# Chemical118/TREW

Measured on AMD Instinct MI355X. Metric: Gbases/s scanned (short 5 32, 150 bp reads), higher is better.
Workload: dtype u32

## Files before the change

### include/trew_hip.h

```cpp
#ifndef TREW_HIP_H
#define TREW_HIP_H

#include <stddef.h>
#include <stdint.h>

#ifdef __cplusplus
extern "C" {
#endif

#define TREW_HIP_ABI_VERSION 4

enum {
    TREW_MODE_SHORT = 0,
    TREW_MODE_PAIR = 1,
    TREW_MODE_LONG = 2,
    TREW_MODE_SEGMENT = 3
};

enum {
    TREW_TABLE_FORWARD_HIGH = 0,
    TREW_TABLE_FORWARD_LOW = 1,
    TREW_TABLE_BACKWARD_HIGH = 2,
    TREW_TABLE_BACKWARD_LOW = 3,
    TREW_TABLE_BOTH_HIGH = 4,
    TREW_TABLE_BOTH_LOW = 5,
    TREW_NUM_TABLES = 6
};

enum {
    TREW_FLAG_NO_FILTER = 1,
    TREW_FLAG_DEBUG_NO_EMIT = 2,
    TREW_FLAG_DEBUG_NO_KLOOP = 4,
    TREW_FLAG_DEBUG_POISON_LDS = 32,
    TREW_FLAG_DEBUG_WIDE_NO_WAIT = 128,
    TREW_FLAG_NO_TIMING = 64,
    TREW_FLAG_COMPAT_G1 = 512,
    TREW_FLAG_DEBUG_NO_JOINT = 2048,
    TREW_FLAG_DEBUG_NO_UNI_DRAIN = 4096,
    TREW_FLAG_DEBUG_NO_GROUP = 1024,
    TREW_FLAG_DEBUG_ANNOT_GENERAL = 8192,
    TREW_FLAG_TRACK_PRESSURE = 256
};

typedef struct {
    int32_t min_mer;
    int32_t max_mer;
    double low_baseline;
    double high_baseline;
    int32_t slice_length;
    int32_t mode;
    int32_t device;
    int32_t n_slots;
    uint64_t max_batch_words;
    uint64_t max_batch_reads;
    uint32_t table_log2_slots;
    uint32_t flags;
    uint64_t max_batch_ascii_bytes;
} trew_hip_params;

typedef struct {
    const uint32_t *words;
    uint64_t n_words;
    const uint32_t *offsets;
    const uint32_t *lengths;
    uint32_t uniform_length;
    uint32_t uniform_stride;
    uint64_t n_reads;
    int32_t on_device;
    int32_t max_length;
} trew_hip_batch;

typedef struct {
    const char *bases;
    uint64_t n_bytes;
    const uint32_t *byte_offsets;
    const uint32_t *lengths;
    const uint32_t *word_offsets;
    uint32_t uniform_length;
    uint32_t reserved;
    uint64_t n_reads;
} trew_hip_ascii_batch;

typedef struct {
    int32_t k;
    int32_t table;
    uint64_t word_lo;
    uint64_t word_hi;
    uint64_t count;
} trew_hip_row;

typedef struct trew_hip_ctx trew_hip_ctx;

int trew_hip_init(const trew_hip_params *params, trew_hip_ctx **out);
void trew_hip_destroy(trew_hip_ctx *ctx);
const char *trew_hip_last_error(const trew_hip_ctx *ctx);

int trew_hip_submit(trew_hip_ctx *ctx, const trew_hip_batch *batch, int slot);
int trew_hip_submit_ascii(trew_hip_ctx *ctx, const trew_hip_ascii_batch *batch, int slot);
int trew_hip_pack_ascii(trew_hip_ctx *ctx, const trew_hip_ascii_batch *batch, uint32_t *words, uint64_t words_cap, uint64_t *n_words);
int trew_hip_wait(trew_hip_ctx *ctx, int slot);

int trew_hip_collect(trew_hip_ctx *ctx, int table, trew_hip_row *rows, uint64_t cap, uint64_t *n_rows);
int trew_hip_reset_tables(trew_hip_ctx *ctx);
int trew_hip_add_rows(trew_hip_ctx *ctx, const trew_hip_row *rows, uint64_t n_rows);

int trew_hip_collect_device(trew_hip_ctx *ctx, trew_hip_row *d_rows, uint64_t cap, uint64_t *n_rows);
int trew_hip_add_rows_device(trew_hip_ctx *ctx, const trew_hip_row *d_rows, uint64_t n_rows);
int trew_hip_merge(trew_hip_ctx *dst, trew_hip_ctx *src);
int trew_hip_add_gathered_device(trew_hip_ctx *ctx, const trew_hip_row *d_buf, uint32_t n_slices, uint32_t own_slice,
                                 uint64_t slice_rows, void *producer_stream, uint64_t *max_rows);
int trew_hip_collect_slice_device(trew_hip_ctx *ctx, trew_hip_row *d_slice, uint64_t slice_rows, void *consumer_stream, uint64_t *n_rows);

int trew_hip_table_pressure(trew_hip_ctx *ctx, uint64_t *used_slots, uint64_t *total_slots, uint64_t *spilled_rows,
                            uint64_t *spill_capacity);

#define TREW_DEBUG_COUNTERS 8
int trew_hip_debug_counters(trew_hip_ctx *ctx, uint64_t *out, int n);

int trew_hip_debug_worklist(trew_hip_ctx *ctx, int slot, uint32_t *units, uint64_t cap, uint64_t *n);

int trew_hip_segment_results(trew_hip_ctx *ctx, int slot, int32_t *k_high, int32_t *k_low,
                             uint64_t *seq_high, uint64_t *seq_low, uint64_t *seq_high_hi, uint64_t *seq_low_hi,
// ... 88 lines not shown
```

### trew_amd/__init__.py

```python
from . import capi
from .capi import (
    FLAG_NO_FILTER,
    FLAG_DEBUG_ANNOT_GENERAL,
    FLAG_DEBUG_POISON_LDS,
    FLAG_NO_TIMING,
    FLAG_TRACK_PRESSURE,
    FLAG_COMPAT_G1,
    FLAG_DEBUG_NO_GROUP,
    FLAG_DEBUG_NO_JOINT,
    FLAG_DEBUG_NO_UNI_DRAIN,
    FLAG_DEBUG_WIDE_NO_WAIT,
    MODE_LONG,
    MODE_PAIR,
    MODE_SEGMENT,
    MODE_SHORT,
    TABLE_NAMES,
    TrewHip,
    TrewHipError,
    annotate,
    intervals,
    k_mer_check,
    pack_reads,
    tracts,
    variants,
)
```

### trew_amd/capi.py

```python
from __future__ import annotations

import ctypes as C
import os

import numpy as np

_HERE = os.path.dirname(os.path.abspath(__file__))
LIB_PATH = os.environ.get("TREW_HIP_LIB") or os.path.join(_HERE, "lib", "libtrew_hip.so")

MODE_SHORT, MODE_PAIR, MODE_LONG, MODE_SEGMENT = 0, 1, 2, 3
FLAG_NO_FILTER = 1
FLAG_DEBUG_POISON_LDS = 32
FLAG_NO_TIMING = 64
FLAG_COMPAT_G1 = 512
FLAG_TRACK_PRESSURE = 256
FLAG_DEBUG_NO_JOINT = 2048
FLAG_DEBUG_NO_UNI_DRAIN = 4096
FLAG_DEBUG_NO_GROUP = 1024
FLAG_DEBUG_ANNOT_GENERAL = 8192
FLAG_DEBUG_WIDE_NO_WAIT = 128
TABLE_NAMES = ("forward_high", "forward_low", "backward_high", "backward_low", "both_high", "both_low")

EXPORTED_SYMBOLS = (
    "trew_hip_init", "trew_hip_destroy", "trew_hip_last_error", "trew_hip_submit", "trew_hip_wait",
    "trew_hip_collect", "trew_hip_reset_tables", "trew_hip_add_rows", "trew_hip_segment_results",
    "trew_hip_filter_masks", "trew_hip_last_timing", "trew_pack_words", "trew_pack_reads",
    "trew_synth_short_ascii", "trew_synth_short_device", "trew_synth_pair_ascii", "trew_synth_pair_device",
    "trew_hip_malloc", "trew_hip_free", "trew_hip_memcpy_h2d", "trew_hip_memcpy_d2h", "trew_hip_abi_version",
    "trew_pack_pairs", "trew_hip_host_alloc", "trew_hip_host_free", "trew_hip_device_count",
    "trew_synth_long_lengths", "trew_synth_long_ascii", "trew_synth_long_device",
    "trew_hip_collect_device", "trew_hip_add_rows_device", "trew_hip_merge", "trew_hip_table_pressure",
    "trew_hip_add_gathered_device", "trew_hip_collect_slice_device", "trew_hip_debug_counters", "trew_hip_debug_worklist", "trew_hip_submit_ascii", "trew_hip_pack_ascii",
    "trew_motif_parse", "trew_hip_annotate", "trew_hip_annotate_results", "trew_annotate_host",
    "trew_hip_tracts", "trew_hip_tracts_results", "trew_tracts_host",
    "trew_hip_intervals", "trew_hip_intervals_results", "trew_intervals_host",
    "trew_hip_variants", "trew_hip_variants_results", "trew_variants_host",
)
DEBUG_COUNTERS = ("strict_rerun", "windows_fallback", "wide_spin_timeout", "inserted", "inserted_wide", "group_punt", "group_routed", "group_target")


class Params(C.Structure):
    _fields_ = [
        ("min_mer", C.c_int32), ("max_mer", C.c_int32),
        ("low_baseline", C.c_double), ("high_baseline", C.c_double),
        ("slice_length", C.c_int32), ("mode", C.c_int32), ("device", C.c_int32), ("n_slots", C.c_int32),
        ("max_batch_words", C.c_uint64), ("max_batch_reads", C.c_uint64),
        ("table_log2_slots", C.c_uint32), ("flags", C.c_uint32),
        ("max_batch_ascii_bytes", C.c_uint64),
    ]


class Batch(C.Structure):
    _fields_ = [
        ("words", C.c_void_p), ("n_words", C.c_uint64),
        ("offsets", C.c_void_p), ("lengths", C.c_void_p),
        ("uniform_length", C.c_uint32), ("uniform_stride", C.c_uint32),
        ("n_reads", C.c_uint64), ("on_device", C.c_int32), ("max_length", C.c_int32),
    ]


class AsciiBatch(C.Structure):
    _fields_ = [
        ("bases", C.c_void_p), ("n_bytes", C.c_uint64),
        ("byte_offsets", C.c_void_p), ("lengths", C.c_void_p), ("word_offsets", C.c_void_p),
        ("uniform_length", C.c_uint32), ("reserved", C.c_uint32), ("n_reads", C.c_uint64),
    ]


class Row(C.Structure):
    _fields_ = [("k", C.c_int32), ("table", C.c_int32), ("word_lo", C.c_uint64), ("word_hi", C.c_uint64),
                ("count", C.c_uint64)]


class Motif(C.Structure):
    _fields_ = [("k", C.c_int32), ("reserved", C.c_int32), ("word", C.c_uint64)]


class Annot(C.Structure):
    _fields_ = [("windows_fwd", C.c_uint32), ("windows_rev", C.c_uint32), ("tract_start_fwd", C.c_uint32),
                ("tract_len_fwd", C.c_uint32), ("tract_start_rev", C.c_uint32), ("tract_len_rev", C.c_uint32)]


ANNOT_DTYPE = np.dtype([(name, "<u4") for name, _ in Annot._fields_])
assert ANNOT_DTYPE.itemsize == C.sizeof(Annot)
MAX_MOTIFS = 8


class Tract(C.Structure):
    _fields_ = [(name + sfx, C.c_uint32) for sfx in ("_fwd", "_rev")
                for name in ("covered", "head_len", "head_cov", "tail_len", "tail_cov")]


TRACT_DTYPE = np.dtype([(name, "<u4") for name, _ in Tract._fields_])
assert TRACT_DTYPE.itemsize == C.sizeof(Tract) == 40


class IntervalRule(C.Structure):
    _fields_ = [("max_gap", C.c_uint32), ("min_len", C.c_uint32)]


class Interval(C.Structure):
# ... 637 lines not shown
```

### trew_amd/csrc/kernels/decide_group.inc

```

#define TREW_REGION_LIST(X) \
    X(chunk) X(stage) X(group_setup) X(bounds) X(group) X(dg_loop) X(dg_pick) X(dg_eval) X(er_gaps) X(er_runs) X(er_canon) X(er_merge) X(er_max) \
    X(dg_decision) X(dg_end) X(routing) X(records) X(target) X(target_rows) X(target_eval) X(target_emit) X(fallback)
#define TREW_REGION_ENUM(n) kRegion_##n,
enum { TREW_REGION_LIST(TREW_REGION_ENUM) kRegionCount };
#ifdef TREW_REGION_COUNTS
__device__ unsigned long long g_region[64];
#define TREW_MARK(n)                                                                   \
    do {                                                                               \
        asm volatile("; MARK " #n);                                                    \
        if (lane_id() == 0) atomicAdd(&g_region[kRegion_##n], 1ull);                   \
    } while (0)
#else
#define TREW_MARK(n) asm volatile("; MARK " #n)
#endif
__device__ __forceinline__ void lds_sync() {
    __builtin_amdgcn_fence(__ATOMIC_RELEASE, "wavefront");
    __builtin_amdgcn_wave_barrier();
    __builtin_amdgcn_fence(__ATOMIC_ACQUIRE, "wavefront");
}
#define TREW_DPP(v, ctrl) ((u32) __builtin_amdgcn_update_dpp(0, (int) (v), (ctrl), 0xf, 0xf, false))
__device__ __forceinline__ u32 swap16(u32 v) { return (u32) __builtin_amdgcn_ds_swizzle((int) v, 0x401F); }
template <int G = 16>
__device__ __forceinline__ u32 row_or(u32 v) {
// ... 3 lines not shown
    v |= TREW_DPP(v, 0x121);
    if (G == 32) v |= swap16(v);
    return v;
}
template <int G = 16>
__device__ __forceinline__ u32 row_add(u32 v) {
    v += TREW_DPP(v, 0x128);
    v += TREW_DPP(v, 0x124);
    v += TREW_DPP(v, 0x122);
    v += TREW_DPP(v, 0x121);
    if (G == 32) v += swap16(v);
    return v;
}
template <int G = 16>
__device__ __forceinline__ u32 row_max(u32 v) {
    v = max(v, TREW_DPP(v, 0x128));
    v = max(v, TREW_DPP(v, 0x124));
    v = max(v, TREW_DPP(v, 0x122));
    v = max(v, TREW_DPP(v, 0x121));
    if (G == 32) v = max(v, swap16(v));
    return v;
}
__device__ __forceinline__ u32 lane_gather(u32 v, u32 src) { return (u32) __builtin_amdgcn_ds_bpermute((int) (src << 2), (int) v); }
__device__ __forceinline__ u64 lane_gather(u64 v, u32 src) { return ((u64) lane_gather((u32) (v >> 32), src) << 32) | lane_gather((u32) v, src); }

template <int NW>
__device__ __forceinline__ u32 pack_bound(const LaneMasks<NW> &m, const DevParams &P) {
    static_assert(NW <= 10, "COUNT must fit 10 bits");
    const u32 runs = m.runs < 127u ? m.runs : 127u;
    return m.m8 | (m.cnt << 10) | (runs << 20) | (m.ub >= P.low ? 1u << 27 : 0u) | (m.ub >= P.high ? 1u << 28 : 0u) | (m.has_n ? 1u << 29 : 0u);
}

__device__ __forceinline__ void group_fill_multiples(ExactSmem sm, const DevParams &P) {
    const u32 i = lane_id();
    if (i < 32u) {
        const int k = P.min_mer + (int) i;
        u32 m = 0;
        for (int t = k; t <= P.min_mer + 31; t += k) m |= 1u << (t - P.min_mer);
        sm_group(sm)[kGroupMult + i] = m;
    }
}

template <int NW>
__device__ __forceinline__ u32 select_bit(const u32 (&m)[NW], u32 r) {
    u32 word = m[0], sub = 0, base = 0, cum = 0;
#pragma unroll
    for (int w = 0; w + 1 < NW; w++) {
        cum += __popc(m[w]);
        const bool ge = r >= cum;
        word = ge ? m[w + 1] : word;
        sub = ge ? cum : sub;
        base = ge ? 32u * (u32) (w + 1) : base;
    }
    r -= sub;
#pragma unroll
    for (u32 sh = 16; sh >= 1; sh >>= 1) {
        const u32 c = __popc(word & ((1u << sh) - 1u));
        const bool ge = r >= c;
        r -= ge ? c : 0u;
        word = ge ? word >> sh : word;
        base += ge ? sh : 0u;
    }
    return base;
}

__device__ __forceinline__ u64 window_word_at(ExactSmem sm, u32 p, int k) {
    const u32 wi = p >> 5, sh = 2u * (p & 31u);
    const u64 a = sm_seq(sm)[wi], b = sm_seq(sm)[wi + 1];
    const u64 x = sh ? ((a << sh) | (b >> (64u - sh))) : a;
    return x >> (64 - 2 * k);
}

template <typename WT>
struct RowCount {
    u32 R;
    u32 over;
    u32 count;
    WT canon;
    u32 cnt;
    u32 maxc;
    u32 homo;
    WT mseq;
};
template <int NW, typename WT, bool WANT_SEQ, int G = 16>
__device__ __forceinline__ RowCount<WT> eval_row(ExactSmem sm, const u32 (&lo)[NW], const u32 (&hi)[NW], const u32 (&v1)[NW], u32 has_n, u32 s0, int k,
                                                 int W, u32 ev) {
    static_assert(G == 16 || G == 32, "a group is a DPP row or half a wave");
    constexpr u32 kGM = G == 32 ? 0xffffffffu : 0xffffu;
    const u32 lane = lane_id(), j = lane & (u32) (G - 1), gbase = lane & (u32) (64 - G);
    RowCount<WT> rc;
    u32 V[NW];
#pragma unroll
    for (int w = 0; w < NW; w++) {
        V[w] = low_mask(W - 32 * w);
    }
    u32 many_n = 0;
    const bool gaps = __any((ev & has_n) != 0u);
    if (gaps) {
        TREW_MARK(er_gaps);
        u32 nn[NW], left = 0;
#pragma unroll
        for (int w = 0; w < NW; w++) {
            nn[w] = (ev & has_n) ? (~v1[w] & low_mask(W + k - 1 - 32 * w)) : 0u;
            left += __popc(nn[w]);
        }
        many_n = left > 4u ? 1u : 0u;
        left = many_n ? 0u : left;
        while (__any(left != 0u)) {
            u32 p = 0, found = 0;
#pragma unroll
            for (int w = 0; w < NW; w++) {
                const u32 here = (found == 0u && nn[w] != 0u) ? 1u : 0u;
                p = here ? 32u * (u32) w + (u32) __builtin_ctz(nn[w] | (here ^ 1u)) : p;
                nn[w] = here ? (nn[w] & (nn[w] - 1u)) : nn[w];
                found |= here;
            }
            const int a = left ? ((int) p - k + 1 > 0 ? (int) p - k + 1 : 0) : 0, b = left ? (int) p + 1 : 0;
#pragma unroll
            for (int w = 0; w < NW; w++) {
                V[w] &= ~(low_mask(b - 32 * w) & ~low_mask(a - 32 * w));
            }
            left = left ? left - 1u : 0u;
        }
    }
    TREW_MARK(er_runs);
    u32 st[NW], E[NW], R = 0, count = 0;
    {
        u32 prev = 0;
#pragma unroll
        for (int w = 0; w < NW; w++) {
            E[w] = ~((lo[w] ^ shr_var_word<NW>(lo, w, (u32) k)) | (hi[w] ^ shr_var_word<NW>(hi, w, (u32) k)));
            const u32 ve = V[w] & E[w];
            st[w] = V[w] & ~((ve << 1) | (prev >> 31));
            prev = ve;
            R += __popc(st[w]);
            count += __popc(V[w]);
        }
    }
    rc.R = R;
    rc.count = count;
    rc.over = ev & ((R > (u32) G ? 1u : 0u) | many_n);
    ev &= rc.over ^ 1u;
    const bool runlane = ev != 0u && j < R;
    const u32 s = runlane ? select_bit<NW>(st, j) : 0u;
    u32 e;
    if (gaps) {
        u32 en[NW];
#pragma unroll
        for (int w = 0; w < NW; w++) {
            const u32 vn = w + 1 < NW ? V[w + 1 < NW ? w + 1 : 0] : 0u;
            en[w] = V[w] & ~(E[w] & alignbit(vn, V[w], 1u));
        }
        e = runlane ? select_bit<NW>(en, j) : 0u;
    } else {
        const u32 nxt = G == 32 ? (u32) __builtin_amdgcn_update_dpp(0, (int) s, 0x130, 0xf, 0xf, true) : (u32) __builtin_amdgcn_update_dpp(0, (int) s, 0x101, 0xf, 0xf, true);
        e = (j + 1u < R) ? nxt - 1u : (u32) (W - 1);
    }
    const u32 len = e - s + 1u;
    WT canon = ~(WT) 0;
    TREW_MARK(er_canon);
    if (runlane) canon = min_rotation<WT>(window_word_at(sm, s0 + s, k), k);
    u32 rem = ev ? (R >= (u32) G ? kGM : ((1u << (R & 31u)) - 1u)) : 0u;
    u32 tot = 0, last = 0, first = 0;
    u32 covered = 0, best = 0;
    while (__any(rem != 0u)) {
        TREW_MARK(er_merge);
        const bool open = ((rem >> j) & 1u) != 0u;
        const u32 lead = rem ? (u32) __builtin_ctz(rem) : 0u;
        const WT other = lane_gather(canon, gbase + lead);
        const bool eq = open && other == canon;
        const u32 bal = (u32) (__ballot(eq) >> gbase) & kGM;
        const u32 total = row_add<G>(eq ? len : 0u);
        const u32 lend = lane_gather(e, gbase + (bal ? 31u - (u32) __builtin_clz(bal) : 0u));
        covered += total;
        best = total > best ? total : best;
        const bool settled = rem != 0u && best > count - covered;
        const bool alone = settled && open && !eq;
        tot = eq ? total : (alone ? len : tot);
        last = eq ? lend : (alone ? e : last);
        first = eq ? (j == lead ? 1u : 0u) : (alone ? 1u : first);
        rem = settled ? 0u : (rem & ~bal);
    }
    TREW_MARK(er_max);
    const u32 key = runlane ? ((tot << 16) | (0xffffu - last)) : 0u;
    const u32 mkey = row_max<G>(key);
    const u32 win = (runlane && key == mkey) ? 1u : 0u;
    rc.maxc = mkey >> 16;
    rc.homo = row_or<G>(win & (is_homopolymer<WT>(canon, k) ? 1u : 0u));
    rc.mseq = 0;
    if (WANT_SEQ) {
        const u32 wb = (u32) (__ballot(win != 0u) >> gbase) & kGM;
        rc.mseq = lane_gather(canon, gbase + (wb ? (u32) __builtin_ctz(wb) : 0u));
    }
    rc.canon = canon;
    rc.cnt = first ? tot : 0u;
    return rc;
}

template <int NW, int G = 16, bool IN_LDS = true>
__device__ __forceinline__ void row_prepare(ExactSmem sm, const ReadRef &rd, const Segment &sg, bool rowvalid) {
    static_assert((64 / G) * 6 * NW <= 128, "the groups' 6 NW words each must fit kGroupBnd's 128 words");
    static_assert(3 * NW <= G, "a lane per (feature, word)");
    const u32 lane = lane_id(), g = lane / (u32) G, j = lane & (u32) (G - 1);
    u32 *prep = sm_group(sm) + kGroupBnd + g * (6u * NW);
    const u32 p = j / (u32) NW, w = j - p * (u32) NW;
    const bool mine = j < 3u * NW && rowvalid;
    u32 lo1[1] = {0}, hi1[1] = {0}, nm1[1] = {0};
    if (mine) {
        if (IN_LDS)
            load_planes_lds<1>(rd, sg.start + 32u * w, lo1, hi1, nm1);
        else
            load_planes<1>(rd, sg.start + 32u * w, lo1, hi1, nm1);
    }
    const u32 v1 = ~nm1[0] & low_mask((int) sg.len - 32 * (int) w);
    const u32 f1 = lo1[0] & v1, f2 = hi1[0] & v1;
    const u32 x = word_parity(p == 0u ? f1 : (p == 1u ? f2 : (f1 & f2)));
    const u32 top = mine ? x >> 31 : 0u;
    u32 carry = 0;
#pragma unroll
    for (int u = 0; u + 1 < NW; u++) {
        const u32 t = lane_gather(top, g * (u32) G + p * (u32) NW + (u32) u);
        carry ^= (u32) u < w ? t : 0u;
    }
    if (mine) {
        prep[j] = p == 0u ? lo1[0] : (p == 1u ? hi1[0] : v1);
        prep[3 * NW + j] = ((x ^ (0u - carry)) << 1) | carry;
    }
}

template <int NW>
struct RowSeg {
    u32 lo[NW], hi[NW], v1[NW], P1[NW], P2[NW], P3[NW];
    u32 has_n;
};
template <int NW, int G = 16>
__device__ __forceinline__ void row_load(ExactSmem sm, int L, RowSeg<NW> &r) {
    const u32 g = lane_id() / (u32) G;
    const u32 *prep = sm_group(sm) + kGroupBnd + g * (6u * NW);
    u32 anyn = 0;
#pragma unroll
    for (int w = 0; w < NW; w++) {
        r.lo[w] = prep[0 * NW + w];
        r.hi[w] = prep[1 * NW + w];
        r.v1[w] = prep[2 * NW + w];
        r.P1[w] = prep[3 * NW + w];
        r.P2[w] = prep[4 * NW + w];
        r.P3[w] = prep[5 * NW + w];
        anyn |= ~r.v1[w] & low_mask(L - 32 * w);
    }
    r.has_n = anyn != 0u ? 1u : 0u;
}

template <int NW, bool SMALLK>
__device__ __forceinline__ u32 shr_k_word(const u32 (&x)[NW], int w, u32 k) {
    if (SMALLK) return alignbit(w + 1 < NW ? x[w + 1 < NW ? w + 1 : 0] : 0u, x[w], k);
    return shr_var_word<NW>(x, w, k);
}
template <int NW, bool SMALLK = false>
__device__ __forceinline__ u32 bound_at_k(const RowSeg<NW> &r, int L, int k, int gmax, const DevParams &P) {
    const u32 ku = (u32) k;
    u32 V[NW];
    windows_without_n<NW>(r.v1, r.has_n != 0u , L, k, 32, V);
    Buckets8<false, false> b8;
    u32 Ew[NW];
#pragma unroll
    for (int w = 0; w < NW; w++) {
        const u32 F1 = r.P1[w] ^ shr_k_word<NW, SMALLK>(r.P1, w, ku), F2 = r.P2[w] ^ shr_k_word<NW, SMALLK>(r.P2, w, ku);
        const u32 F3 = r.P3[w] ^ shr_k_word<NW, SMALLK>(r.P3, w, ku);
        Ew[w] = ~((r.lo[w] ^ shr_k_word<NW, SMALLK>(r.lo, w, ku)) | (r.hi[w] ^ shr_k_word<NW, SMALLK>(r.hi, w, ku)));
        b8.add(F1, F2, F3, V[w]);
    }
    const u32 m8 = b8.largest(), count = b8.count, links = class_links<NW>(V, Ew);
    const u32 runs = count - links < 127u ? count - links : 127u;
    const double dm = (double) m8, dc = (double) count;
    const double tl = P.low * dc, th = P.high * dc;
    u32 pass_lo = dm > tl ? 1u : 0u, pass_hi = dm > th ? 1u : 0u;
    const bool amb = fabs(dm - tl) <= 1e-9 || fabs(dm - th) <= 1e-9;
    if (__any(amb)) {
        const double ub = count ? dm / dc : 0.0;
        pass_lo = ub >= P.low ? 1u : 0u;
        pass_hi = ub >= P.high ? 1u : 0u;
    }
    const bool inr = k <= gmax && count != 0u;
    return inr ? (m8 | (count << 10) | (runs << 20) | (pass_lo << 27) | (pass_hi << 28) | (r.has_n << 29)) : (r.has_n << 29);
}

template <typename WT>
struct GroupOut {
    u32 kk;
    WT sh, sl;
    u32 saved;
    WT kept_canon;
    u32 kept_cnt;
    bool punt;
};

template <int NW, typename WT, bool WANT_SEQ, int G = 16>
__device__ __forceinline__ GroupOut<WT> decide_group(ExactSmem sm, const DevParams &P, const RowSeg<NW> &rs, u32 bnd0, u32 bnd1, u32 range, const Segment &sg,
                                                     bool valid) {
    static_assert(sizeof(WT) == 8, "k <= 32: the k range must fit a 32-bit index mask");
    PH_T0(t_ph);
    const u32 lane = lane_id(), j = lane & (u32) (G - 1), gbase = lane & (u32) (64 - G);
    const u32 *grp = sm_group(sm);
    const u32 (&lo)[NW] = rs.lo;
    const u32 (&hi)[NW] = rs.hi;
    const int L = (int) sg.len;
    const u32 s0 = range_base(sm, range) + sg.start;
    const u32 has_n = rs.has_n;
    GroupOut<WT> o;
    o.kk = 0;
    o.sh = o.sl = 0;
    o.saved = 0;
    o.kept_canon = 0;
    o.kept_cnt = 0;
    u32 todo = 0;
    {
        const u32 a = (u32) (sg.kmin - P.min_mer) & 31u, b = (u32) (sg.kmax - P.min_mer);
        const u32 m = (b >= 31u ? 0xffffffffu : ((2u << (b & 31u)) - 1u)) & ~((1u << a) - 1u);
        todo = (valid && sg.kmax >= sg.kmin) ? m : 0u;
    }
    u32 lo_num = 0, lo_den = 0, hi_num = 0, hi_den = 0, closed_lo = 0, closed_hi = 0;
    u32 sk0 = 0, sk1 = 0, skb0 = 0, skb1 = 0, skm0 = 0, skm1 = 0;
    u32 viol = 0, punt = 0;
    const u32 m8_0 = bnd0 & 1023u, cn_0 = (bnd0 >> 10) & 1023u, m8_1 = bnd1 & 1023u, cn_1 = (bnd1 >> 10) & 1023u;
    const u32 bit0 = 1u << j, bit1 = G == 16 ? 1u << ((16u + j) & 31u) : 0u;
    auto eligible = [&]() __attribute__((always_inline)) -> u32 {
        const u32 l0 = (bnd0 >> 27) & ~(closed_lo >> j) & (__umul24(m8_0, lo_den) >= __umul24(lo_num, cn_0) ? 1u : 0u);
        const u32 h0 = (bnd0 >> 28) & ~(closed_hi >> j) & (__umul24(m8_0, hi_den) >= __umul24(hi_num, cn_0) ? 1u : 0u);
        if (G == 32) return row_or<G>(((l0 | h0) & 1u) ? bit0 : 0u);
        const u32 l1 = (bnd1 >> 27) & ~(closed_lo >> ((16u + j) & 31u)) & (__umul24(m8_1, lo_den) >= __umul24(lo_num, cn_1) ? 1u : 0u);
        const u32 h1 = (bnd1 >> 28) & ~(closed_hi >> ((16u + j) & 31u)) & (__umul24(m8_1, hi_den) >= __umul24(hi_num, cn_1) ? 1u : 0u);
        return row_or<G>((((l0 | h0) & 1u) ? bit0 : 0u) | (((l1 | h1) & 1u) ? bit1 : 0u));
    };
    TREW_MARK(dg_loop);
    todo &= eligible();
    for (;;) {
        u32 act, kidx, bk;
        for (;;) {
            TREW_MARK(dg_pick);
            act = (todo != 0u && punt == 0u) ? 1u : 0u;
            kidx = act ? (u32) __builtin_ctz(todo) : 0u;
            bk = G == 32 ? lane_gather(bnd0, gbase + kidx) : lane_gather(kidx >= 16u ? bnd1 : bnd0, gbase + (kidx & 15u));
            const u32 heavy = act & (((bk >> 20) & 127u) > (u32) G ? 1u : 0u);
            if (!__any(heavy)) break;
            const u32 m8k = bk & 1023u, cntk = (bk >> 10) & 1023u;
            const u32 el = ((bk >> 27) & ~(closed_lo >> kidx) & (__umul24(m8k, lo_den) >= __umul24(lo_num, cntk) ? 1u : 0u) & 1u) |
                           (((bk >> 28) & ~(closed_hi >> kidx) & (__umul24(m8k, hi_den) >= __umul24(hi_num, cntk) ? 1u : 0u) & 1u) << 1);
            const u32 mk = grp[kGroupMult + kidx];
            const u32 take0 = heavy & (sk0 == 0u ? 1u : 0u), take1 = heavy & (take0 ^ 1u) & (sk1 == 0u ? 1u : 0u);
            sk0 = take0 ? (kidx | (el << 8) | (1u << 12)) : sk0;
            skb0 = take0 ? (m8k | (cntk << 16)) : skb0;
            skm0 = take0 ? mk : skm0;
            sk1 = take1 ? (kidx | (el << 8) | (1u << 12)) : sk1;
            skb1 = take1 ? (m8k | (cntk << 16)) : skb1;
            skm1 = take1 ? mk : skm1;
            punt |= heavy & ((take0 | take1) ^ 1u);
            todo = heavy ? (todo & (todo - 1u)) : todo;
        }
        if (!__any(act)) break;
        TREW_MARK(dg_eval);
        todo &= todo - 1u;
        const int k = P.min_mer + (int) kidx;
        const u32 lo_open = ~(closed_lo >> kidx) & 1u, hi_open = ~(closed_hi >> kidx) & 1u;
        u32 ev = act;
        const int W = ev ? L - k + 1 : 1;
        PH_T0(t_runs);
        const RowCount<WT> rc = eval_row<NW, WT, WANT_SEQ, G>(sm, lo, hi, rs.v1, has_n, s0, k, W, ev);
        punt |= rc.over;
        ev &= rc.over ^ 1u;
        const u32 R = rc.R, maxc = rc.maxc, count = rc.count, homo = rc.homo;
        const WT mseq = rc.mseq, canon = rc.canon;
        PH_ADD(PH_RUNS, t_runs);
        TREW_MARK(dg_decision);
        const double dm = (double) maxc, dc = (double) count;
        const double tl = P.low * dc, th = P.high * dc;
        u32 base_lo = dm > tl ? 1u : 0u, base_hi = dm > th ? 1u : 0u;
        if (__any(ev != 0u && (fabs(dm - tl) <= 1e-9 || fabs(dm - th) <= 1e-9))) {
            const double f = dm / dc;
            base_lo = f >= P.low ? 1u : 0u;
            base_hi = f >= P.high ? 1u : 0u;
        }
        const u32 ge_lo = lo_den ? (__umul24(maxc, lo_den) >= __umul24(lo_num, count) ? 1u : 0u) : base_lo;
        const u32 ge_hi = hi_den ? (__umul24(maxc, hi_den) >= __umul24(hi_num, count) ? 1u : 0u) : base_hi;
        const u32 okv = ev & (homo ^ 1u) & (maxc != 0u ? 1u : 0u);
        const u32 acc_lo = okv & lo_open & ge_lo, acc_hi = okv & hi_open & ge_hi, acc = acc_lo | (acc_hi << 1);
        const u32 mk = grp[kGroupMult + kidx];
        o.kk = acc_lo ? ((o.kk & 0xffu) | ((u32) k << 8)) : o.kk;
        o.kk = acc_hi ? ((o.kk & 0xff00u) | (u32) k) : o.kk;
        lo_num = acc_lo ? maxc : lo_num;
        lo_den = acc_lo ? count : lo_den;
        hi_num = acc_hi ? maxc : hi_num;
        hi_den = acc_hi ? count : hi_den;
        closed_lo |= acc_lo ? mk : 0u;
        closed_hi |= acc_hi ? mk : 0u;
        if (WANT_SEQ) {
            o.sl = acc_lo ? mseq : o.sl;
            o.sh = acc_hi ? mseq : o.sh;
        }
        o.saved = acc ? ((u32) k | (R << 8) | (count << 16)) : o.saved;
        o.kept_canon = acc ? canon : o.kept_canon;
        o.kept_cnt = acc ? rc.cnt : o.kept_cnt;
        {
            const u32 hit0 = acc & (sk0 >> 8) & 3u, hit1 = acc & (sk1 >> 8) & 3u;
            const u32 bad0 = (__umul24(maxc, skb0 >> 16) < __umul24(skb0 & 0xffffu, count) ? 1u : 0u) | ((skm0 >> kidx) & 1u);
            const u32 bad1 = (__umul24(maxc, skb1 >> 16) < __umul24(skb1 & 0xffffu, count) ? 1u : 0u) | ((skm1 >> kidx) & 1u);
            viol |= (hit0 ? bad0 : 0u) | (hit1 ? bad1 : 0u);
            sk0 |= hit0 << 10;
            sk1 |= hit1 << 10;
        }
        if (__any(acc)) {
            todo &= eligible();
            if (!__any(todo != 0u && punt == 0u)) break;
        }
    }
    TREW_MARK(dg_end);
    viol |= ((sk0 >> 8) & 3u & ~((sk0 >> 10) & 3u)) | ((sk1 >> 8) & 3u & ~((sk1 >> 10) & 3u));
    o.punt = (punt | viol) != 0u;
    PH_ADD(PH_DECIDE, t_ph);
    return o;
}

__device__ __forceinline__ void stage_two(ExactSmem sm, const ReadRef &rdA, const ReadRef &rdB, bool haveB) {
    const u32 lane = lane_id();
    lds_sync();
    const u32 r = lane >> 5, segwords = exact_rangewords(sm.cap);
    ReadRef rr;
    rr.w = r ? rdB.w : rdA.w;
    rr.len = r ? rdB.len : rdA.len;
    rr.nw = r ? rdB.nw : rdA.nw;
    const u32 L = rr.len;
    u64 *seq = sm_seq(sm) + r * segwords;
    u32 *nmk = sm_nmask(sm) + r * segwords;
    const u32 nwords = (L + 31u) >> 5;
    if (r == 0u || haveB) {
        for (u32 l = lane & 31u; l < segwords; l += 32u) {
            u64 sq = 0;
            u32 nmv = 0xffffffffu;
            if (l < nwords) {
                u32 lo1[1], hi1[1], nm1[1];
                load_planes_lds<1>(rr, 32u * l, lo1, hi1, nm1);
                nmv = nm1[0] | ~low_mask<true>((int) L - 32 * (int) l);
                const u32 lq = lo1[0] & ~nmv, hq = hi1[0] & ~nmv;
                sq = spread32(__brev(lq)) | (spread32(__brev(hq)) << 1);
            }
            seq[l] = sq;
            nmk[l] = nmv;
        }
    }
    lds_sync();
}

template <typename WT>
__device__ __forceinline__ WT strand_canon(WT w, int k) {
    const WT rc = min_rotation<WT>(revcomp(w, k), k);
    return rc < w ? rc : w;
}

template <typename WT>
__device__ __forceinline__ WT strand_flip(WT w, int k) {
    return min_rotation<WT>(revcomp(w, k), k);
}

template <int NW, typename WT>
__device__ void run_short_group(ExactSmem sm, const DevParams &P, TableRef T, const ReadRef rdA, const ReadRef rdB, bool haveB) {
    const u32 lane = lane_id();
#if defined(TREW_AB_SKIP) && TREW_AB_SKIP >= 5
    return;
#endif
    TREW_MARK(stage);
    PH_T0(t_stage);
    stage_two(sm, rdA, rdB, haveB);
    PH_ADD(PH_STAGE, t_stage);
#if defined(TREW_AB_SKIP) && TREW_AB_SKIP >= 4
    return;
#endif
    TREW_MARK(group_setup);
    const u32 g = lane >> 4, j = lane & 15u;
    const bool second = g >= 2u;
    const u32 is_right = g & 1u;
    ReadRef rd;
    rd.w = second ? rdB.w : rdA.w;
    rd.len = second ? rdB.len : rdA.len;
    rd.nw = second ? rdB.nw : rdA.nw;
    const Segment sg = get_segment(TREW_MODE_SHORT, (int) is_right, rd.len, 0, P.min_mer, P.max_mer, P.slice_len);
    const bool rowvalid = sg.valid && (!second || haveB);
    TREW_MARK(bounds);
    PH_T0(t_bounds);
    lds_sync();
    row_prepare<NW>(sm, rd, sg, rowvalid);
    lds_sync();
    RowSeg<NW> rs;
    row_load<NW>(sm, (int) sg.len, rs);
    u32 bnd0;
    if (P.min_mer + 15 < 32)
        bnd0 = rowvalid ? bound_at_k<NW, true>(rs, (int) sg.len, P.min_mer + (int) j, P.max_mer, P) : 0u;
    else
        bnd0 = rowvalid ? bound_at_k<NW, false>(rs, (int) sg.len, P.min_mer + (int) j, P.max_mer, P) : 0u;
    const u32 bnd1 = rowvalid ? bound_at_k<NW>(rs, (int) sg.len, P.min_mer + 16 + (int) j, P.max_mer, P) : 0u;
#if defined(TREW_AB_SKIP) && TREW_AB_SKIP >= 3
    asm volatile("" ::"v"(bnd0), "v"(bnd1));
    return;
#endif
    PH_ADD(PH_BOUNDS, t_bounds);
    TREW_MARK(group);
    const GroupOut<WT> o = decide_group<NW, WT, false>(sm, P, rs, bnd0, bnd1, second ? 1u : 0u, sg, rowvalid);
#if defined(TREW_AB_SKIP) && TREW_AB_SKIP >= 2
    asm volatile("" ::"v"(o.kk), "v"(o.saved), "v"(o.kept_cnt), "v"((u32) o.kept_canon), "v"((u32) (o.kept_canon >> 32)), "v"((u32) o.punt));
    return;
#endif
    TREW_MARK(routing);
    PH_T0(t_route);
    const u32 mine = rowvalid ? (o.kk | (o.punt ? 1u << 16 : 0u)) : 0u;
    const u32 other = lane_gather(mine, lane ^ 16u);
    const u32 kkL = is_right ? other : mine, kkR = is_right ? mine : other;
    const u32 lkh = kkL & 255u, lkl = (kkL >> 8) & 255u, rkh = kkR & 255u, rkl = (kkR >> 8) & 255u;
    const u32 left_found = (lkh | lkl) != 0u ? 1u : 0u;
    const u32 tgt_h = left_found & (lkh == rkh ? 1u : 0u) & (lkh != 0u ? 1u : 0u);
    const u32 tgt_l = left_found & (lkl == rkl ? 1u : 0u) & (lkl != 0u ? 1u : 0u);
    const u32 myk = o.saved & 255u, items = (o.saved >> 8) & 255u;
    u32 need_old = ((kkL | kkR) >> 16) & 1u;
    u32 rec_mask = 0;
    {
        const u32 kh = is_right ? rkh : lkh, kl = is_right ? rkl : lkl;
        const u32 rec_h = (kh != 0u ? 1u : 0u) & (is_right ? ((left_found ^ 1u) | (lkh == 0u ? 1u : 0u)) : (tgt_h ^ 1u));
        const u32 rec_l = (kl != 0u ? 1u : 0u) & (is_right ? ((left_found ^ 1u) | (lkl == 0u ? 1u : 0u)) : (tgt_l ^ 1u));
        const u32 th = is_right ? (1u << TREW_TABLE_BACKWARD_HIGH) : (1u << TREW_TABLE_FORWARD_HIGH);
        const u32 tl = is_right ? (1u << TREW_TABLE_BACKWARD_LOW) : (1u << TREW_TABLE_FORWARD_LOW);
        rec_mask = ((rec_h & (kh == myk ? 1u : 0u)) ? th : 0u) | ((rec_l & (kl == myk ? 1u : 0u)) ? tl : 0u);
        need_old |= (rec_h & (kh != myk ? 1u : 0u)) | (rec_l & (kl != myk ? 1u : 0u));
    }
    need_old |= tgt_h & tgt_l & (lkh != lkl ? 1u : 0u);
    {
        const u32 hh = (lkh == 0u && rkh == 0u) ? 1u : 0u, lh = (lkl == 0u && rkl == 0u) ? 1u : 0u;
        const Segment sW = get_segment(TREW_MODE_SHORT, 2, rd.len, 0, P.min_mer, P.max_mer, P.slice_len);
        need_old |= (sW.valid ? 1u : 0u) & (hh | lh);
    }
    need_old |= lane_gather(need_old, lane ^ 16u);
    need_old &= rowvalid ? 1u : 0u;
    const DevTable Tv = load_table(T);
    TREW_MARK(records);
    if (need_old == 0u && rec_mask != 0u && j < items && o.kept_cnt != 0u) {
        for (u32 tm = rec_mask; tm; tm &= tm - 1u) cached_add(sm, Tv, __ffs((int) tm) - 1, (int) myk, o.kept_canon, o.kept_cnt);
    }
    PH_ADD(PH_EMIT, t_route);
    TREW_MARK(target);
    PH_T0(t_target);
    u32 want_t = (need_old ^ 1u) & (tgt_h | tgt_l) & (rowvalid ? 1u : 0u);
    {
        const int tk = (int) (tgt_h ? lkh : lkl);
        const u32 rowbase = lane & 48u;
        const u32 cnt = (j < items) ? o.kept_cnt : 0u;
        const u32 c1 = row_max<16>(cnt);
        const u32 topb = (u32) (__ballot(cnt != 0u && cnt == c1) >> rowbase) & 0xffffu;
        const u32 tl = topb ? (u32) __builtin_ctz(topb) : 0u;
        const u32 c2 = (o.saved >> 16) - c1;
        const WT xkey = lane_gather(o.kept_canon, rowbase + tl);
        const u32 okrow = want_t & (myk == (u32) tk ? 1u : 0u) & (c1 != 0u ? 1u : 0u) & (o.punt ? 0u : 1u);
        const u32 pc1 = lane_gather(c1, lane ^ 16u), pc2 = lane_gather(c2, lane ^ 16u), pok = lane_gather(okrow, lane ^ 16u);
        const u32 pcount = lane_gather(o.saved >> 16, lane ^ 16u);
        const WT pkey = lane_gather(xkey, lane ^ 16u);
        const u32 fast = okrow & pok & (xkey == pkey ? 1u : 0u) & (c1 + pc1 > c2 + pc2 + (u32) (tk - 1) ? 1u : 0u);
        if (__any(fast != 0u)) {
            TREW_MARK(target_rows);
            const u32 q = lane & 31u, r = second ? 1u : 0u, segwords = exact_rangewords(sm.cap);
            const int i = (int) (rd.len >> 1) - tk + 1 + (int) q;
            u32 sv = 0;
            WT cs = 0;
            if (fast != 0u && q + 1u < (u32) tk) {
                const u32 *nmk = sm_nmask(sm) + r * segwords;
                const u32 wi = (u32) i >> 5;
                const u32 nb = alignbit(wi + 1u < segwords ? nmk[wi + 1u] : 0xffffffffu, nmk[wi], (u32) i & 31u);
                if ((nb & low_mask<true>(tk)) == 0u) {
                    sv = 1u;
                    cs = min_rotation<WT>(window_word_at(sm, range_base(sm, r) + (u32) i, tk), tk);
                }
            }
            const u32 halfbase = lane & 32u;
            const u32 nspan = (u32) __popc((u32) (__ballot(sv != 0u) >> halfbase));
            const u32 sx = (u32) __popc((u32) (__ballot(sv != 0u && cs == xkey) >> halfbase));
            const u32 maxc = c1 + pc1 + sx, count = (o.saved >> 16) + pcount + nspan;
            const double f = is_homopolymer<WT>(xkey, tk) ? 0.0 : (double) maxc / (double) count;
            const u32 tm = fast ? (((tgt_h && f >= P.high) ? 1u << TREW_TABLE_BOTH_HIGH : 0u) | ((tgt_l && f >= P.low) ? 1u << TREW_TABLE_BOTH_LOW : 0u)) : 0u;
            const bool lead = is_right == 0u && j == tl;
            const u32 add = (cnt != 0u && o.kept_canon == xkey) ? (lead ? maxc : 0u) : cnt;
            if (tm != 0u && add != 0u) {
                const WT w = strand_canon<WT>(o.kept_canon, tk);
                for (u32 t2 = tm; t2; t2 &= t2 - 1u) cached_add(sm, Tv, __ffs((int) t2) - 1, tk, w, add);
            }
            if (tm != 0u && sv != 0u && cs != xkey) {
                const WT w = strand_canon<WT>(cs, tk);
                for (u32 t2 = tm; t2; t2 &= t2 - 1u) cached_add(sm, Tv, __ffs((int) t2) - 1, tk, w, 1u);
            }
        }
        want_t &= fast ^ 1u;
    }
    u32 tgt_old = 0;
    if (__any(want_t != 0u)) {
        constexpr int NWW = 2 * NW;
        const u32 ev = want_t & (is_right ^ 1u);
        const int tk = (int) (tgt_h ? lkh : lkl);
        u32 wlo[NWW], whi[NWW], wv1[NWW], w_n = 0;
        {
            u32 nm[NWW];
            ReadRef r = rd;
            if (!ev) r.nw = 0;
            load_planes_lds<NWW>(r, 0, wlo, whi, nm);
#pragma unroll
            for (int w = 0; w < NWW; w++) {
                const u32 lm = low_mask((int) rd.len - 32 * w);
                wv1[w] = ~nm[w] & lm;
                w_n |= nm[w] & lm;
            }
        }
        const int W = ev ? (int) rd.len - tk + 1 : 1;
        TREW_MARK(target_eval);
        const RowCount<WT> rc = eval_row<NWW, WT, false>(sm, wlo, whi, wv1, w_n != 0u ? 1u : 0u, range_base(sm, second ? 1u : 0u), ev ? tk : P.min_mer, W, ev);
        TREW_MARK(target_emit);
        tgt_old = rc.over;
        const u32 okc = ev & (rc.over ^ 1u);
        const double f = rc.homo ? 0.0 : (double) rc.maxc / (double) rc.count;
        const u32 tm = ((tgt_h && f >= P.high) ? 1u << TREW_TABLE_BOTH_HIGH : 0u) | ((tgt_l && f >= P.low) ? 1u << TREW_TABLE_BOTH_LOW : 0u);
        if (okc != 0u && tm != 0u && rc.cnt != 0u) {
            const WT w = strand_canon<WT>(rc.canon, tk);
            for (u32 t2 = tm; t2; t2 &= t2 - 1u) cached_add(sm, Tv, __ffs((int) t2) - 1, tk, w, rc.cnt);
        }
    }
    PH_ADD(PH_RECORD_EVAL, t_target);
    TREW_MARK(fallback);
    const u64 ob = __ballot(need_old != 0u), tb = __ballot(tgt_old != 0u);
    if ((ob | tb) == 0ull) return;
    __syncthreads();
    if (!o.punt && j < items) {
        sm_save_canon<WT>(sm)[g * kSaveItems + j] = o.kept_canon;
        sm_save_cnt<WT>(sm)[g * kSaveItems + j] = (unsigned short) o.kept_cnt;
    }
    if (j == 0u) put_decision<WT>(sm, g, o.kk | (o.punt ? 1u << 16 : 0u), o.saved, o.sh, o.sl);
    const u64 pb = __ballot(o.punt && rowvalid);
    const u64 thb = __ballot(tgt_h != 0u), tlb = __ballot(tgt_l != 0u);
    const u32 tkA = (u32) __builtin_amdgcn_readlane((int) (tgt_h ? lkh : lkl), 0), tkB = (u32) __builtin_amdgcn_readlane((int) (tgt_h ? lkh : lkl), 32);
    __syncthreads();
    for (u32 r = 0; r < (haveB ? 2u : 1u); r++) {
        const ReadRef &rr = r ? rdB : rdA;
        if ((ob >> (32u * r)) & 1ull) {
            const u32 punted = ((pb >> (32u * r)) & 1ull ? 1u : 0u) | ((pb >> (32u * r + 16u)) & 1ull ? 2u : 0u);
            if (punted) {
                count_fallback(kFallbackGroupPunt);
                decide_halves<NW, WT>(sm, P, rr, r, 2u * r, punted);
            }
            count_fallback(kFallbackGroupRouted);
            run_short_routed<NW, WT>(sm, P, T, rr, r, 2u * r, true);
            __syncthreads();
        } else if ((tb >> (32u * r)) & 1ull) {
            count_fallback(kFallbackGroupTarget);
            target<WT>(view_segment(sm, r, 0, rr), P, T, (int) rr.len, (int) (r ? tkB : tkA), ((thb >> (32u * r)) & 1ull) != 0ull, ((tlb >> (32u * r)) & 1ull) != 0ull);
            __syncthreads();
        }
    }
}
```

### trew_amd/csrc/kernels/exact_kernel.inc

```

#ifndef TREW_EXACT_SHORT_WAVES
#define TREW_EXACT_SHORT_WAVES 5
#endif
#ifndef TREW_EXACT_PAIR_WAVES
#define TREW_EXACT_PAIR_WAVES 4
#endif
#ifndef TREW_EXACT_LONG_WAVES
#define TREW_EXACT_LONG_WAVES 4
#endif
template <int NW, int MODE>
constexpr int exact_waves(bool narrow) {
    return NW >= 10 ? 4
                    : (narrow && NW > 0 && MODE == TREW_MODE_SHORT
                           ? TREW_EXACT_SHORT_WAVES
                           : (narrow && NW > 0 && MODE == TREW_MODE_PAIR ? TREW_EXACT_PAIR_WAVES : (narrow && NW == 5 && MODE == TREW_MODE_LONG ? TREW_EXACT_LONG_WAVES : 6)));
}
template <int NW, int MODE, typename WT>
__global__ __launch_bounds__(64, (exact_waves<NW, MODE>(sizeof(WT) == 8))) void exact_kernel(DevParams P, DevBatch B, DevTableG1 TG, const u32 *wl,
                                                   u32 *wl_count, u32 *wl_count_next, u32 wl_cap, SegResults R, u32 cap, u32 rawwords) {
    struct KernArgs {
        DevParams P;
        DevBatch B;
        DevTableG1 TG;
    };
// ... 83 lines not shown
            u32 *meta = meta_base + bf * kMetaWords;
            const bool mine = lane < nit * kPer;
            const u64 read_l = mine ? (u64) meta[lane / kPer] * kPer + lane % kPer : 0ull;
            u64 off_l = 0;
            u32 len_l = 0;
            if (mine) {
                off_l = Bk.offsets ? (u64) Bk.offsets[read_l] : read_l * (u64) Bk.uniform_stride;
                len_l = Bk.lengths ? Bk.lengths[read_l] : Bk.uniform_length;
            }
            if (lane < kChunk) {
                meta[4 + lane] = len_l;
                meta[8 + lane] = (u32) off_l;
                meta[12 + lane] = (u32) (off_l >> 32);
                meta[16 + lane] = 3u * ((len_l + 31u) >> 5) <= sm.rawwords ? 1u : 0u;
            }
#pragma unroll
            for (u32 t = 0; t < kChunk; t++) {
                const u64 off = readlane_word(off_l, (int) t);
                const u32 nwords = 3u * (((u32) __builtin_amdgcn_readlane((int) len_l, (int) t) + 31u) >> 5);
                if (nwords <= sm.rawwords) {
                    u32 *dst = raw_base + (bf * kChunk + t) * sm.rawwords;
                    for (u32 j0 = 0; j0 < nwords; j0 += 64u)
                        if (j0 + lane < nwords) __builtin_amdgcn_global_load_lds(Bk.words + off + j0 + lane, (__attribute__((address_space(3))) u32 *) (dst + j0), 4, 0, 0);
                }
            }
        };
        auto landed = [&]() __attribute__((always_inline)) {
            __builtin_amdgcn_s_waitcnt(0);
            __syncthreads();
        };
        u32 bf = 0;
        PH_T0(t_stage0);
        issue_claim();
        u64 cur = resolve_claim();
        if (cur != ~0ull) {
            fetch_units(0, cur, chunk_items(cur));
            landed();
            fetch_words(0, chunk_items(cur));
            issue_claim();
            landed();
        }
        PH_ADD(PH_STAGE, t_stage0);
        constexpr bool kGroup = MODE == TREW_MODE_SHORT && sizeof(WT) == 8 && (NW == 3 || NW == 5);
        bool grouped = false;
        if constexpr (kGroup) grouped = use_group;
        while (cur != ~0ull) {
            TREW_MARK(chunk);
            const u32 nit = chunk_items(cur);
            u32 *const meta = meta_base + bf * kMetaWords;
            PH_T0(t_p0);
            const u64 nxt = resolve_claim();
            PH_ADD(PH_STAGE, t_p0);
            const u32 nxt_nit = nxt != ~0ull ? chunk_items(nxt) : 0u;
            if (nxt_nit) fetch_units(bf ^ 1u, nxt, nxt_nit);
            const u32 hook = nit < kUnits / 2u ? nit : kUnits / 2u;
            PH_CNT(PH_N_READS, nit);
            auto item = [&](u32 t, ReadRef &rd, u32 &unit, bool &staged) __attribute__((always_inline)) {
                rd.len = rfl(meta[4 + t]);
                rd.nw = (rd.len + 31u) >> 5;
                unit = rfl(meta[t / kPer]);
                const u64 off = ((u64) rfl(meta[12 + t]) << 32) | rfl(meta[8 + t]);
                staged = rfl(meta[16 + t]) != 0u;
                rd.w = staged ? (const u32 *) (raw_base + (bf * kChunk + t) * sm.rawwords) : B.words + off;
            };
            ReadRef held;
            held.w = nullptr;
            held.len = held.nw = 0;
            bool have_held = false;
            for (u32 t = 0; t <= nit; t++) {
                if (t == hook && nxt_nit) {
                    PH_T0(t_p1);
                    landed();
                    PH_ADD(PH_STAGE, t_p1);
                    fetch_words(bf ^ 1u, nxt_nit);
                    issue_claim();
                }
                if constexpr (MODE == TREW_MODE_PAIR) {
                    if (t < nit) {
                        ReadRef r0, r1;
                        u32 unit = 0, unit1 = 0;
                        bool st0, st1;
                        item(2u * t, r0, unit, st0);
                        item(2u * t + 1u, r1, unit1, st1);
                        run_pair<NW, WT>(sm, P, T, unit, r0, r1);
                        __syncthreads();
                    }
                    continue;
                }
                ReadRef rd;
                rd.w = nullptr;
                rd.len = rd.nw = 0;
                u32 unit = 0;
                bool ok = false;
                if (t < nit) {
                    bool staged;
                    item(t, rd, unit, staged);
                    ok = grouped && staged && 4 * P.min_mer <= (int) rd.len;
                    if (!ok) {
                        if (MODE == TREW_MODE_SHORT)
                            run_short<NW, WT>(sm, P, T, rd);
                        else
                            run_segment<NW, WT>(sm, P, T, unit, rd, R);
                        __syncthreads();
                        continue;
                    }
                }
                if constexpr (kGroup) {
                    if (ok && !have_held) {
                        held = rd;
                        have_held = true;
                    } else if (have_held) {
                        ReadRef second = held;
                        if (ok) second = rd;
                        run_short_group<NW, WT>(sm, P, T, held, second, ok);
                        have_held = false;
                    }
                }
            }
            PH_T0(t_p2);
            if (nxt_nit) landed();
            PH_ADD(PH_STAGE, t_p2);
            cur = nxt;
            bf ^= 1u;
        }
    } else if (MODE == TREW_MODE_LONG && sizeof(WT) == 8 && NW == 5 && use_group) {
        if constexpr (MODE == TREW_MODE_LONG && sizeof(WT) == 8 && NW == 5) run_long_groups<NW, WT>(sm, P, B, T, wl, heads, n);
    } else {
        for (u32 attempt = 0; attempt < kShards; attempt++) {
            const u32 sh = (my + attempt) & (kShards - 1);
            for (;;) {
                u32 c = 0;
                if (lane == 0) c = atomicAdd(&heads[sh * kHeadStride], 1u);
                c = rfl(c);
                const u64 w0l = ((u64) c * kShards + sh) * kChunk;
                if (w0l >= n) break;
                const u32 w0 = (u32) w0l;
                const u32 nit = (w0 + kChunk < n ? w0 + kChunk : n) - w0;
                u32 units[kChunk];
#pragma unroll
                for (u32 t = 0; t < kChunk; t++) units[t] = t < nit ? wl[w0 + t] : 0u;
#pragma unroll
                for (u32 t = 0; t < kChunk; t++) {
                    if (t < nit) {
                        if constexpr (MODE == TREW_MODE_LONG) run_long<NW, WT>(sm, P, B, T, units[t]);
                        __syncthreads();
                    }
                }
            }
        }
    }
    {
        PH_T0(t_flush);
        cache_flush(sm, T);
        PH_ADD(PH_FLUSH, t_flush);
    }
    PH_ADD(PH_TOTAL, t_total);
#ifdef TREW_PHASE_PROFILE
    __syncthreads();
    if (lane_id() < 32) atomicAdd(&g_phase[lane_id()], ph_lds()[lane_id()]);
#endif
}

#ifdef TREW_REGION_COUNTS
extern "C" int trew_debug_regions(unsigned long long *out, int n, int reset) {
    unsigned long long v[64];
    if (hipMemcpyFromSymbol(v, HIP_SYMBOL(g_region), sizeof(v)) != hipSuccess) return 1;
    for (int i = 0; i < n && i < 64; i++) out[i] = v[i];
// ... 22 lines not shown
```

Before: 1997.

## Replace iterative run merge with fixed-distance DPP merge and N-free bound specialization

When every active row has few runs, eval_row replaces the iterative ballot-driven merge loop over equal canonical runs with an unrolled sequence of DPP row shifts that compare each run's canonical word with neighbours up to a fixed distance. bound_at_k gains a specialization for reads with no N bases: window masks and the count are computed directly, and for NW==3 with short windows the top word is skipped. A debug flag keeps the old reference path. run_pair is force-inlined for wide word types, which may raise register pressure.

```diff
diff --git a/include/trew_hip.h b/include/trew_hip.h
--- a/include/trew_hip.h
+++ b/include/trew_hip.h
@@ -38,6 +38,7 @@
     TREW_FLAG_DEBUG_NO_JOINT = 2048,
     TREW_FLAG_DEBUG_NO_UNI_DRAIN = 4096,
     TREW_FLAG_DEBUG_NO_GROUP = 1024,
+    TREW_FLAG_DEBUG_ROW_REFERENCE = 16384,
     TREW_FLAG_DEBUG_ANNOT_GENERAL = 8192,
     TREW_FLAG_TRACK_PRESSURE = 256
 };
diff --git a/trew_amd/__init__.py b/trew_amd/__init__.py
--- a/trew_amd/__init__.py
+++ b/trew_amd/__init__.py
@@ -9,6 +9,7 @@
     FLAG_DEBUG_NO_GROUP,
     FLAG_DEBUG_NO_JOINT,
     FLAG_DEBUG_NO_UNI_DRAIN,
+    FLAG_DEBUG_ROW_REFERENCE,
     FLAG_DEBUG_WIDE_NO_WAIT,
     MODE_LONG,
     MODE_PAIR,
diff --git a/trew_amd/capi.py b/trew_amd/capi.py
--- a/trew_amd/capi.py
+++ b/trew_amd/capi.py
@@ -17,6 +17,7 @@
 FLAG_DEBUG_NO_JOINT = 2048
 FLAG_DEBUG_NO_UNI_DRAIN = 4096
 FLAG_DEBUG_NO_GROUP = 1024
+FLAG_DEBUG_ROW_REFERENCE = 16384
 FLAG_DEBUG_ANNOT_GENERAL = 8192
 FLAG_DEBUG_WIDE_NO_WAIT = 128
 TABLE_NAMES = ("forward_high", "forward_low", "backward_high", "backward_low", "both_high", "both_low")
diff --git a/trew_amd/csrc/kernels/decide_group.inc b/trew_amd/csrc/kernels/decide_group.inc
--- a/trew_amd/csrc/kernels/decide_group.inc
+++ b/trew_amd/csrc/kernels/decide_group.inc
@@ -109,9 +109,43 @@
     u32 homo;
     WT mseq;
 };
+#ifndef TREW_ROW_MERGE_D
+#define TREW_ROW_MERGE_D 8
+#endif
+constexpr int kRowMergeD = TREW_ROW_MERGE_D;
+static_assert(kRowMergeD >= 2 && kRowMergeD <= 16, "distances inside a DPP row");
+template <int R>
+__device__ __forceinline__ u32 row_from_below(u32 v) { return (u32) __builtin_amdgcn_update_dpp(0, (int) v, 0x110 + R, 0xf, 0xf, true); }
+template <int R>
+__device__ __forceinline__ u32 row_from_above(u32 v) { return (u32) __builtin_amdgcn_update_dpp(0, (int) v, 0x100 + R, 0xf, 0xf, true); }
+template <int R>
+__device__ __forceinline__ void merge_distance(u32 clo, u32 chi, u32 len, u32 e, u32 runlane, u32 j, u32 runs, u32 &tot, u32 &last, u32 &lower) {
+    const u32 blo = row_from_below<R>(clo), bhi = row_from_below<R>(chi), ldn = row_from_below<R>(len);
+    const u32 alo = row_from_above<R>(clo), ahi = row_from_above<R>(chi), lup = row_from_above<R>(len), eup = row_from_above<R>(e);
+    const u32 dn = runlane & (j >= (u32) R ? 1u : 0u) & (((blo ^ clo) | (bhi ^ chi)) == 0u ? 1u : 0u);
+    const u32 up = runlane & (j + (u32) R < runs ? 1u : 0u) & (((alo ^ clo) | (ahi ^ chi)) == 0u ? 1u : 0u);
+    tot += (dn ? ldn : 0u) + (up ? lup : 0u);
+    last = up ? eup : last;
+    lower |= dn;
+}
+template <int R, int D>
+struct MergeDistances {
+    template <typename ANY>
+    static __device__ __forceinline__ void run(u32 clo, u32 chi, u32 len, u32 e, u32 runlane, u32 j, u32 runs, const ANY &more, u32 &tot, u32 &last, u32 &lower) {
+        if (!more(R)) return;
+        merge_distance<R>(clo, chi, len, e, runlane, j, runs, tot, last, lower);
+        MergeDistances<R + 1, D>::run(clo, chi, len, e, runlane, j, runs, more, tot, last, lower);
+    }
+};
+template <int D>
+struct MergeDistances<D, D> {
+    template <typename ANY>
+    static __device__ __forceinline__ void run(u32, u32, u32, u32, u32, u32, u32, const ANY &, u32 &, u32 &, u32 &) {}
+};
+
 template <int NW, typename WT, bool WANT_SEQ, int G = 16>
 __device__ __forceinline__ RowCount<WT> eval_row(ExactSmem sm, const u32 (&lo)[NW], const u32 (&hi)[NW], const u32 (&v1)[NW], u32 has_n, u32 s0, int k,
-                                                 int W, u32 ev) {
+                                                 int W, u32 ev, bool row_ref) {
     static_assert(G == 16 || G == 32, "a group is a DPP row or half a wave");
     constexpr u32 kGM = G == 32 ? 0xffffffffu : 0xffffu;
     const u32 lane = lane_id(), j = lane & (u32) (G - 1), gbase = lane & (u32) (64 - G);
@@ -189,6 +223,16 @@
     if (runlane) canon = min_rotation<WT>(window_word_at(sm, s0 + s, k), k);
     u32 rem = ev ? (R >= (u32) G ? kGM : ((1u << (R & 31u)) - 1u)) : 0u;
     u32 tot = 0, last = 0, first = 0;
+    if (G == 16 && sizeof(WT) == 8 && !row_ref && !__any(ev != 0u && R > (u32) kRowMergeD)) {
+        TREW_MARK(er_merge);
+        u32 lower = 0;
+        tot = runlane ? len : 0u;
+        last = e;
+        const auto more = [&](int r) __attribute__((always_inline)) { return __any(ev != 0u && R > (u32) r) != 0; };
+        MergeDistances<1, kRowMergeD>::run((u32) canon, (u32) ((u64) canon >> 32), len, e, runlane ? 1u : 0u, j, R, more, tot, last, lower);
+        first = runlane ? lower ^ 1u : 0u;
+        rem = 0;
+    }
     u32 covered = 0, best = 0;
     while (__any(rem != 0u)) {
         TREW_MARK(er_merge);
@@ -283,21 +327,28 @@
     if (SMALLK) return alignbit(w + 1 < NW ? x[w + 1 < NW ? w + 1 : 0] : 0u, x[w], k);
     return shr_var_word<NW>(x, w, k);
 }
-template <int NW, bool SMALLK = false>
+template <int NW, bool SMALLK = false, int NC = NW, bool NFREE = false>
 __device__ __forceinline__ u32 bound_at_k(const RowSeg<NW> &r, int L, int k, int gmax, const DevParams &P) {
+    static_assert(NC == NW || (NFREE && NC < NW), "words are only left out where the windows are known");
     const u32 ku = (u32) k;
-    u32 V[NW];
-    windows_without_n<NW>(r.v1, r.has_n != 0u , L, k, 32, V);
-    Buckets8<false, false> b8;
-    u32 Ew[NW];
-#pragma unroll
-    for (int w = 0; w < NW; w++) {
+    u32 V[NC];
+    if constexpr (NFREE) {
+#pragma unroll
+        for (int w = 0; w < NC; w++) V[w] = low_mask(L - k + 1 - 32 * w);
+    } else {
+        windows_without_n<NW>(r.v1, r.has_n != 0u , L, k, 32, V);
+    }
+    Buckets8<false, NFREE> b8;
+    u32 Ew[NC];
+#pragma unroll
+    for (int w = 0; w < NC; w++) {
         const u32 F1 = r.P1[w] ^ shr_k_word<NW, SMALLK>(r.P1, w, ku), F2 = r.P2[w] ^ shr_k_word<NW, SMALLK>(r.P2, w, ku);
         const u32 F3 = r.P3[w] ^ shr_k_word<NW, SMALLK>(r.P3, w, ku);
         Ew[w] = ~((r.lo[w] ^ shr_k_word<NW, SMALLK>(r.lo, w, ku)) | (r.hi[w] ^ shr_k_word<NW, SMALLK>(r.hi, w, ku)));
         b8.add(F1, F2, F3, V[w]);
     }
-    const u32 m8 = b8.largest(), count = b8.count, links = class_links<NW>(V, Ew);
+    const u32 count = NFREE ? (u32) (L - k + 1 > 0 ? L - k + 1 : 0) : b8.count;
+    const u32 m8 = b8.largest(count), links = class_links<NC>(V, Ew);
     const u32 runs = count - links < 127u ? count - links : 127u;
     const double dm = (double) m8, dc = (double) count;
     const double tl = P.low * dc, th = P.high * dc;
@@ -392,7 +443,7 @@
         u32 ev = act;
         const int W = ev ? L - k + 1 : 1;
         PH_T0(t_runs);
-        const RowCount<WT> rc = eval_row<NW, WT, WANT_SEQ, G>(sm, lo, hi, rs.v1, has_n, s0, k, W, ev);
+        const RowCount<WT> rc = eval_row<NW, WT, WANT_SEQ, G>(sm, lo, hi, rs.v1, has_n, s0, k, W, ev, (P.flags & TREW_FLAG_DEBUG_ROW_REFERENCE) != 0u);
         punt |= rc.over;
         ev &= rc.over ^ 1u;
         const u32 R = rc.R, maxc = rc.maxc, count = rc.count, homo = rc.homo;
@@ -518,12 +569,23 @@
     lds_sync();
     RowSeg<NW> rs;
     row_load<NW>(sm, (int) sg.len, rs);
-    u32 bnd0;
-    if (P.min_mer + 15 < 32)
-        bnd0 = rowvalid ? bound_at_k<NW, true>(rs, (int) sg.len, P.min_mer + (int) j, P.max_mer, P) : 0u;
+    const int L = (int) sg.len;
+#ifdef TREW_AB_PLAIN_BOUNDS
+    const bool plain = true;
+#else
+    const bool plain = (P.flags & TREW_FLAG_DEBUG_ROW_REFERENCE) != 0u || P.min_mer + 15 >= 32 || __any(rowvalid && rs.has_n != 0u);
+#endif
+    u32 bnd0, bnd1;
+    if (!plain)
+        bnd0 = rowvalid ? bound_at_k<NW, true, NW, true>(rs, L, P.min_mer + (int) j, P.max_mer, P) : 0u;
+    else if (P.min_mer + 15 < 32)
+        bnd0 = rowvalid ? bound_at_k<NW, true>(rs, L, P.min_mer + (int) j, P.max_mer, P) : 0u;
     else
-        bnd0 = rowvalid ? bound_at_k<NW, false>(rs, (int) sg.len, P.min_mer + (int) j, P.max_mer, P) : 0u;
-    const u32 bnd1 = rowvalid ? bound_at_k<NW>(rs, (int) sg.len, P.min_mer + 16 + (int) j, P.max_mer, P) : 0u;
+        bnd0 = rowvalid ? bound_at_k<NW, false>(rs, L, P.min_mer + (int) j, P.max_mer, P) : 0u;
+    if (NW == 3 && !plain && !__any(rowvalid && L - (P.min_mer + 16) + 1 > 64))
+        bnd1 = rowvalid ? bound_at_k<NW, false, (NW == 3 ? 2 : NW), true>(rs, L, P.min_mer + 16 + (int) j, P.max_mer, P) : 0u;
+    else
+        bnd1 = rowvalid ? bound_at_k<NW>(rs, L, P.min_mer + 16 + (int) j, P.max_mer, P) : 0u;
 #if defined(TREW_AB_SKIP) && TREW_AB_SKIP >= 3
     asm volatile("" ::"v"(bnd0), "v"(bnd1));
     return;
@@ -641,7 +703,8 @@
         }
         const int W = ev ? (int) rd.len - tk + 1 : 1;
         TREW_MARK(target_eval);
-        const RowCount<WT> rc = eval_row<NWW, WT, false>(sm, wlo, whi, wv1, w_n != 0u ? 1u : 0u, range_base(sm, second ? 1u : 0u), ev ? tk : P.min_mer, W, ev);
+        const RowCount<WT> rc = eval_row<NWW, WT, false>(sm, wlo, whi, wv1, w_n != 0u ? 1u : 0u, range_base(sm, second ? 1u : 0u), ev ? tk : P.min_mer, W, ev,
+                                                        (P.flags & TREW_FLAG_DEBUG_ROW_REFERENCE) != 0u);
         TREW_MARK(target_emit);
         tgt_old = rc.over;
         const u32 okc = ev & (rc.over ^ 1u);
diff --git a/trew_amd/csrc/kernels/exact_kernel.inc b/trew_amd/csrc/kernels/exact_kernel.inc
--- a/trew_amd/csrc/kernels/exact_kernel.inc
+++ b/trew_amd/csrc/kernels/exact_kernel.inc
@@ -189,7 +189,10 @@
                         bool st0, st1;
                         item(2u * t, r0, unit, st0);
                         item(2u * t + 1u, r1, unit1, st1);
-                        run_pair<NW, WT>(sm, P, T, unit, r0, r1);
+                        if constexpr (sizeof(WT) == 8 && (NW == 3 || NW == 5))
+                            [[clang::always_inline]] run_pair<NW, WT>(sm, P, T, unit, r0, r1);
+                        else
+                            run_pair<NW, WT>(sm, P, T, unit, r0, r1);
                         __syncthreads();
                     }
                     continue;
```

New measurement: 1997, median of 2. No clear change (+0.0%).
